# Villen-Lab/pyAscore

Measured on AMD Instinct MI355X. Metric: PSMs/sec (Ascore.score) at 1/2/4/8 MI355X + HBM-roofline %, higher is better.
Workload: dtype f32/f64 scalar + i32 counts

## Files before the change

pyascore_amd/csrc/common.h:

```cpp
#ifndef PYA_COMMON_H
#define PYA_COMMON_H

#include <stdint.h>

#define PYA_WAVE 64
#define PYA_NTOP 10
#define PYA_NTOP_MAX 16
#define PYA_NO_MATCH 15
#define PYA_TABLE_PAD 4
#define PYA_MAX_L 64
#define PYA_MAX_TYPES 8
#define PYA_MAX_NL 8
#define PYA_FAST_NL 4
#define PYA_MAX_UNIQ_WIDE 48
#define PYA_MAX_NL_CANDS 44
#define PYA_MAX_UNIQ 16
#define PYA_MAX_LIST 2048
#define PYA_MAX_LUT_N 4096
#define PYA_MAX_PUSHED 128

#define PYA_ST_OK 0
#define PYA_ST_NO_BINS 1
#define PYA_ST_TOO_MANY_BINS 2
#define PYA_ST_LUT_RANGE 3
#define PYA_ST_PUSHED_OVERFLOW 4
#define PYA_ST_ROUTE_CAPS 5
#define PYA_ST_INVALID 16
#define PYA_ST_OVER_LIMIT 17

struct PcCaps {
    uint32_t cap, pos_cap, kc, k_cap, n_cap;
};
// ... 117 lines not shown
```

pyascore_amd/csrc/fused_core.hip.h:

```cpp
#ifndef PYA_FUSED_CORE_H
#define PYA_FUSED_CORE_H
#include "score_core.hip.h"
#include "localize_core.hip.h"

#define FUSED_ROUND 3

struct FusedLds {
    uint16_t *grid;
    uint4 *cum_lut;
    PeakEntry *peaks;
    float2 *resd;
    uint8_t *rkl;
    uint32_t *rec;
    float *wsl;
    float *mass_l;
    uint32_t *flag_l;
    uint8_t *site_pos;
    float *selm;
    unsigned char *sort_raw;
    PushedEntry *pushed;
    unsigned long long *site_alt;
    uint32_t *site_max, *site_tie, *n_pushed;
    float *sc;
    uint32_t *c_tr, *c_cnt;
// ... 2 lines not shown
    float *srt_v;
    uint8_t *srt_h;
    int32_t *c_depth;
    uint32_t *c_site;
};

__host__ __device__ static inline size_t fused_align16(size_t v) { return (v + 15) & ~(size_t)15; }
__host__ __device__ static inline size_t fused_sort_bytes(uint32_t n) {
    if (n <= 64) return ((size_t)n * 10 + 15) & ~(size_t)15;
    return (((size_t)n * 6 + 15) & ~(size_t)15) + ((size_t)n / 64 + 2) * 16 + 2 * 128 * 2;
}
__host__ __device__ static inline uint32_t fused_site_cap(uint32_t push_cap) {
    const uint32_t v = (push_cap + 3u) & ~3u;
    return v > 64u ? 64u : (v < 4u ? 4u : v);
}
__host__ __device__ static inline size_t fused_post_bytes(uint32_t n_cap, uint32_t push_cap, uint32_t ent_cap, uint32_t ndir,
                                                          bool multi_z) {
    return fused_align16(fused_sort_bytes(n_cap)) + (size_t)push_cap * 16 + (size_t)fused_site_cap(push_cap) * 16 + 16 +
           (size_t)(1 + FUSED_ROUND) * 40 + (size_t)FUSED_ROUND * (16 * ndir + 4 + 4) + 16 + 64 +
           (multi_z ? fused_align16((size_t)FUSED_ROUND * ndir * 2 * ent_cap * 4) +
                          fused_align16((size_t)FUSED_ROUND * ndir * 2 * ent_cap)
                    : 0);
}
__host__ __device__ static inline size_t fused_walk_bytes(uint32_t cap) {
    return 16 * 16 + ((size_t)cap + PYA_TABLE_PAD) * 8;
}
__host__ __device__ static inline size_t fused_kept_bytes(uint32_t n_cap, uint32_t stride, uint32_t pos_cap, uint32_t ent_cap,
                                                          uint32_t ndir) {
    return fused_align16(((size_t)pos_cap + 1) * 8) + fused_align16((size_t)ent_cap * stride) + (size_t)n_cap * 16 + 256 +
           fused_align16((size_t)pos_cap + 1) + (size_t)(1 + FUSED_ROUND) * ndir * ent_cap * 4;
}
__host__ __device__ static inline size_t fused_lds_bytes(uint32_t cap, uint32_t n_cap, uint32_t stride, uint32_t pos_cap,
                                                         uint32_t ent_cap, uint32_t push_cap, uint32_t ndir, bool multi_z) {
    const size_t walk = fused_walk_bytes(cap), post = fused_post_bytes(n_cap, push_cap, ent_cap, ndir, multi_z);
    return PYA_GRID_CELLS * 2 + fused_align16(walk > post ? walk : post) +
           fused_kept_bytes(n_cap, stride, pos_cap, ent_cap, ndir) + 16;
}

DEV FusedLds fused_carve(unsigned char *raw, uint32_t cap, uint32_t n_cap, uint32_t stride, uint32_t pos_cap,
                         uint32_t ent_cap, uint32_t push_cap, uint32_t ndir, bool multi_z) {
    FusedLds f;
    f.grid = (uint16_t *)raw;
    size_t o = PYA_GRID_CELLS * 2;
    f.cum_lut = (uint4 *)(raw + o);
    f.peaks = (PeakEntry *)(raw + o + 16 * 16);
    f.sort_raw = raw + o;
    size_t q = o + fused_align16(fused_sort_bytes(n_cap));
    f.pushed = (PushedEntry *)(raw + q);
    q += (size_t)push_cap * sizeof(PushedEntry);
    const size_t sc = fused_site_cap(push_cap);
    f.site_alt = (unsigned long long *)(raw + q);
    q += sc * 8;
    f.site_max = (uint32_t *)(raw + q);
    q += sc * 4;
    f.site_tie = (uint32_t *)(raw + q);
    q += sc * 4;
    f.n_pushed = (uint32_t *)(raw + q);
    q += 16;
    f.sc = (float *)(raw + q);
    q += (size_t)(1 + FUSED_ROUND) * 40;
    f.c_tr = (uint32_t *)(raw + q);
    q += (size_t)FUSED_ROUND * ndir * 8;
    f.c_cnt = (uint32_t *)(raw + q);
    q += (size_t)FUSED_ROUND * ndir * 8;
    f.c_depth = (int32_t *)(raw + q);
    q += FUSED_ROUND * 4;
    f.c_site = (uint32_t *)(raw + q);
    q += FUSED_ROUND * 4;
    f.bad_tasks = (uint32_t *)(raw + q);
    q += 16;
    f.t_lo = (uint32_t *)(raw + q);
    f.t_off = f.t_lo + 8;
    q += 64;
    f.srt_v = (float *)(raw + q);
    q += fused_align16((size_t)FUSED_ROUND * ndir * 2 * ent_cap * 4);
    f.srt_h = (uint8_t *)(raw + q);
    const size_t walk = fused_walk_bytes(cap), post = fused_post_bytes(n_cap, push_cap, ent_cap, ndir, multi_z);
    o += fused_align16(walk > post ? walk : post);
    f.resd = (float2 *)(raw + o);
    o += fused_align16(((size_t)pos_cap + 1) * 8);
    f.rkl = (uint8_t *)(raw + o);
    o += fused_align16((size_t)ent_cap * stride);
    f.rec = (uint32_t *)(raw + o);
    o += (size_t)n_cap * 12;
    f.wsl = (float *)(raw + o);
    o += (size_t)n_cap * 4;
    f.mass_l = (float *)(raw + o);
    f.flag_l = (uint32_t *)(raw + o + 128);
    f.site_pos = (uint8_t *)(raw + o + 256);
    f.selm = (float *)(raw + o + 256 + fused_align16((size_t)pos_cap + 1));
    return f;
}


template <bool BZ>
DEV void walk_record_steps(const float2 *&rp, int rstride, StepBits &bits, float &running, const uint4 *lut, CumCounts &cum,
                           const PeakTable &tab, int zmax, double A, double B, uint8_t *&ro, int stride, int count) {
    for (int i = 0; i < count; i++, rp += rstride) {
        const float2 mm = *rp;
        running = (bits.next() ? mm.y : mm.x) + running;
// ... 86 lines not shown
DEV int partners_in_run(const float *run, int n, int p2, float me, int side, float err) {
    int j = 0;
    for (int step = p2 >> 1; step > 0; step >>= 1) {
        const int probe = j + step;
        const float o = probe - 1 < n ? run[probe - 1] : __builtin_huge_valf();
        const float dd = side ? (o - me) : (me - o);
        if (side ? (dd <= -err) : (dd >= err)) j = probe;
    }
    int cnt = 0;
    for (int q = j; q < j + 2 && q < n; q++) {
        const float dd = side ? (run[q] - me) : (me - run[q]);
        cnt += (__builtin_fabsf(dd) < err) ? 1 : 0;
    }
    return cnt;
}

#define FUSED_LOCAL_CHUNKS 8
struct LocalTable {
    const float *mz;
    const uint8_t *rank;
    int R, status;
};

template <bool BOTH, bool ZM, bool WIDE = false>
DEV bool fused_body(const BatchDev &b, uint32_t psm, unsigned char *lds_raw, uint32_t cap, uint32_t n_cap, uint32_t stride,
                    uint32_t pos_cap, uint32_t ent_cap, uint32_t push_cap, const LocalTable *local = nullptr) {
    const int lane = lane_id();
    const DevConfig *cfg = b.cfg;
    const int ndir = BOTH ? 2 : 1;
    const FusedLds f = fused_carve(lds_raw, cap, n_cap, stride, pos_cap, ent_cap, push_cap, (uint32_t)ndir, ZM);
    STAMP_BEGIN();
    STAMP_T(b, 38, false);
    float lmz[FUSED_LOCAL_CHUNKS];
    uint32_t lrk[FUSED_LOCAL_CHUNKS];
    if (local) {
#pragma unroll
        for (int q = 0; q < FUSED_LOCAL_CHUNKS; q++) {
            const int i = q * 64 + lane_id();
            lmz[q] = i < local->R ? local->mz[i] : __builtin_huge_valf();
            lrk[q] = i < local->R ? (uint32_t)local->rank[i] : (uint32_t)PYA_NO_MATCH;
        }
        wave_lds_sync();
    }
    if (lane < 32) {
        f.mass_l[lane] = cfg->res_mass[lane];
        f.flag_l[lane] = cfg->res_modifiable[lane];
    }
    const uint64_t *dw = b.desc + (size_t)psm * PYA_DESC_WORDS;
    const int64_t p0 = (int64_t)dw[0], pep0 = (int64_t)dw[1], s0 = (int64_t)dw[2], a0 = (int64_t)dw[3];
    const uint64_t w4 = dw[4], w5 = dw[5];
    const int L = (int)(w4 & 0xffffu), n_aux = (int)((w4 >> 16) & 0xffffu), k = (int)((w4 >> 32) & 0xffffu);
    const int zmax = ZM ? (int)(w4 >> 56) : 1;
    const int N = (int)(uint32_t)w5;
    const uint64_t *order = b.order_tab + (uint32_t)(w5 >> 32);
    const int status = local ? local->status : b.status[psm];
    const int R = local ? local->R : (int)b.ret_n[psm];

    const uint32_t max_k = b.max_k;
    float *out_asc = b.ascores + (size_t)psm * max_k;
    uint64_t *out_alt = b.alt_mask + (size_t)psm * max_k;
    for (uint32_t a = lane; a < max_k; a += 64) {
        out_asc[a] = 0.f;
        out_alt[a] = 0ull;
    }
    if (status != PYA_ST_OK) {
        if (lane == 0) {
            b.best_score[psm] = -1.f;
            b.best_sig[psm] = 0ull;
            b.n_sig_out[psm] = -1;
        }
        return false;
    }
    STAMP_T(b, 39, false);
    const bool two_pass = BOTH && WIDE && N > 32;
    const int s = (BOTH && !two_pass) ? (lane & 31) : lane;
    const int dir = BOTH ? (two_pass ? 0 : (lane >> 5)) : (cfg->n_fwd > 0 ? 0 : 1);
    const bool active = s < N;
    const uint32_t letter = lane < L ? (uint32_t)b.pep[pep0 + lane] : (uint32_t)'A';
    const uint64_t bits = active ? order[s] : 0ull;
// ... 541 lines not shown
```

pyascore_amd/csrc/host_internal.h:

```cpp
#ifndef PYA_HOST_INTERNAL_H
#define PYA_HOST_INTERNAL_H
#include <hip/hip_runtime_api.h>

#include <algorithm>
#include <atomic>
#include <cmath>
#include <cstdarg>
#include <cstddef>
#include <cstdio>
#include <cstdlib>
#include <chrono>
#include <cstring>
#include <condition_variable>
#include <functional>
#include <map>
#include <memory>
#include <mutex>
#include <string>
#include <thread>
#include <unordered_map>
#include <vector>

#include "../../include/pyascore_hip.h"
#include "common.h"
// ... 31 lines not shown
                   uint32_t use_fused, uint32_t f_n_cap, uint32_t f_stride, uint32_t f_ent_cap, uint32_t f_push_cap,
                   uint32_t multi_z, int32_t *host_status, uint32_t *host_flag, hipStream_t stream);
int pya_launch_ambiguity(const BatchDev *b, uint32_t psm, uint32_t peak_cap, uint32_t list_cap,
                         uint64_t ref_bits, uint64_t oth_bits, const float *d_scores, float ref_ws,
                         float oth_ws, float *d_out, hipStream_t stream);
int pya_launch_debug_sort(const float *d_keys, uint32_t n, uint32_t *d_perm, hipStream_t stream);
int pya_launch_pack_records(const float *best_score, const int32_t *n_sig, const uint64_t *best_sig, const float *ascores,
                            const uint64_t *alt_mask, uint32_t k, uint32_t res_k, uint64_t n_psm, int32_t *out, hipStream_t stream);
int pya_launch_debug_wave_ops(const int32_t *d_in, int32_t *d_out, hipStream_t stream);
size_t pya_score_big_lds_bytes(uint32_t cap, uint32_t pos_cap, uint32_t kc);
int pya_launch_score_big(const BatchDev *b, const uint32_t *d_ids, uint32_t n_ids, uint32_t cap, uint32_t pos_cap, uint32_t kc,
                         uint32_t inline_on, hipStream_t stream);
size_t pya_localize_recount_lds_bytes(uint32_t cap, uint32_t push_cap, uint32_t pos_cap, uint32_t pool_cap, uint32_t sb);
size_t pya_localize_hash_lds_bytes(uint32_t push_cap, uint32_t n_cap, uint32_t pos_cap, uint32_t sb, uint32_t vc, uint32_t hs,
                                   uint32_t pp, uint32_t max_k, uint32_t n_nl);
int pya_launch_localize_hash(const BatchDev *b, const uint32_t *d_ids, uint32_t n_ids, uint32_t push_cap, uint32_t n_cap,
                             uint32_t pos_cap, uint32_t pool_cap, uint32_t sb, uint32_t gtp, uint32_t vc, uint32_t hs, uint32_t pp,
                             uint32_t n_nl, hipStream_t stream);
int pya_launch_localize_recount(const BatchDev *b, const uint32_t *d_ids, uint32_t n_ids, uint32_t cap, uint32_t push_cap,
                                uint32_t pos_cap, uint32_t pool_cap, uint32_t sb, uint32_t gtp, uint32_t *d_redo_count, uint32_t *d_redo_ids, hipStream_t stream);
int pya_launch_score_big_list(const BatchDev *b, const uint32_t *d_count, const uint32_t *d_ids, uint32_t n_max, uint32_t cap,
                              uint32_t pos_cap, uint32_t kc, hipStream_t stream);
uint32_t pya_big_inline_max(void);
size_t pya_fused_lds_bytes(uint32_t cap, uint32_t n_cap, uint32_t stride, uint32_t pos_cap, uint32_t ent_cap, uint32_t push_cap,
                           uint32_t both, uint32_t multi_z);
int pya_launch_fused(const BatchDev *b, const uint32_t *d_ids, uint32_t n_ids, uint32_t cap, uint32_t n_cap,
                     uint32_t stride, uint32_t pos_cap, uint32_t ent_cap, uint32_t push_cap, uint32_t both,
                     uint32_t multi_z, uint32_t *d_redo_count, uint32_t *d_redo_ids, hipStream_t stream);
size_t pya_score_cnt_lds_bytes(uint32_t cap, uint32_t pos_cap, uint32_t kc, uint32_t k_cap, uint32_t n_cap);
int pya_launch_score_cnt(const BatchDev *b, const uint32_t *d_ids, uint32_t n_ids, uint32_t cap, uint32_t pos_cap, uint32_t kc, uint32_t k_cap,
                         uint32_t n_cap, hipStream_t stream);
size_t pya_score_cntg_lds_bytes(uint32_t cap, uint32_t pos_cap, uint32_t k_cap, uint32_t n_cap, uint32_t nl_cap);
int pya_launch_score_cntg(const BatchDev *b, const uint32_t *d_ids, uint32_t n_ids, uint32_t cap, uint32_t pos_cap, uint32_t k_cap, uint32_t n_cap,
                          uint32_t nl_cap, hipStream_t stream);
size_t pya_bin_global_scratch_bytes(uint32_t cap);
int pya_launch_bin_global(const BatchDev *b, const uint32_t *d_ids, uint32_t n_ids, unsigned char *d_scratch, uint64_t stride,
                          uint32_t cap, uint32_t types, hipStream_t stream);
size_t pya_general_lds_bytes(uint32_t l_cap, uint32_t list_cap);
size_t pya_general_scratch_bytes(uint32_t n_cap, uint32_t push_cap);
int pya_launch_general(const BatchDev *b, const uint32_t *d_ids, uint32_t n_ids, unsigned char *d_scratch, const uint64_t *d_scratch_off,
                       uint32_t l_cap, uint32_t list_cap, hipStream_t stream);
int pya_launch_general_ambiguity(const BatchDev *b, uint32_t psm, uint32_t l_cap, uint32_t list_cap, uint64_t ref_bits,
                                 uint64_t oth_bits, const float *d_scores, uint32_t n_scores, float ref_ws, float oth_ws,
                                 float *d_out, hipStream_t stream);
size_t pya_evidence_lds_bytes(uint32_t l_cap, uint32_t list_cap);
int pya_launch_evidence(const BatchDev *b, const uint32_t *d_ids, uint32_t n_ids, void *d_out, uint32_t l_cap, uint32_t list_cap,
                        hipStream_t stream);
size_t pya_ions_lds_bytes(uint32_t l_cap, uint32_t list_cap);
uint32_t pya_ions_scan_tiles(uint32_t n);
int pya_launch_ions(const BatchDev *b, const uint32_t *d_ids, uint32_t n_ids, const void *d_evid, int64_t *d_off, void *d_out, uint64_t cap,
// ... 128 lines not shown
        case 'C': return 103.00919f;  case 'L': return 113.08406f;  case 'I': return 113.08406f;
        case 'N': return 114.04293f;  case 'D': return 115.02694f;  case 'Q': return 128.05858f;
        case 'K': return 128.09496f;  case 'E': return 129.04259f;  case 'M': return 131.04049f;
        case 'H': return 137.05891f;  case 'F': return 147.06841f;  case 'U': return 150.95364f;
        case 'R': return 156.10111f;  case 'Y': return 163.06333f;  case 'W': return 186.07931f;
        case 'O': return 237.14773f;
    }
    return 0.f;
}


struct Knobs {
    bool no_plain = false, no_fused = false, no_big = false, no_tiny = false, no_prefix = false, no_chunks = false;
    bool no_upload_thread = false, one_peak_class = false, peak_classes = false, one_lds_class = false;
    bool host_timing = false, stamps = false, sort_room = false, no_big_inline = false;
    bool no_loc_hash = false, no_nodes = false, no_cnt = false, no_prob_cnt = false;
    bool no_fork = false;
    bool slow_null_stream = false;
    uint32_t debug = 0;
    int64_t plain_min = 512, big_min_n = 1024, tiny_max = 64;
    int64_t bin_select_min = 640;
    int64_t bin_select_scap = 768;
    uint32_t sort_room_max = 1024;
    int sb = -1, gtp = -1, hash_pp = -1;
    int node_cap = -1;
    double chunk_mb = 0.;
    int64_t workspace_mb = 0;
};

void read_knobs(Knobs &k);
bool set_knob(Knobs &k, const char *key, const char *value);

struct pya_handle {
    Knobs kn;
    int device = 0;
    hipStream_t side_stream = nullptr;
    float bin_size = 100.f, mod_mass = 0.f, mz_error = 0.5f;
    uint32_t n_top = PYA_NTOP;
    uint32_t rec_words() const { return (n_top + 1u) / 2u + 1u; }
    std::string mod_group, fragment_types;
    std::map<char, float> nl;
    DevConfig cfg;
    bool cfg_dirty = true;
    DevBuf<DevConfig> d_cfg;

    std::vector<float> lut;
// ... 287 lines not shown
    DevBuf<uint32_t> d_sret_n;
    DevBuf<int32_t> d_sstatus;
    uint64_t spec(uint64_t i) const { return spec_of.empty() ? i : spec_of[i]; }
    int64_t n_peaks(uint64_t i) const {
        const uint64_t s = spec(i);
        return peak_off[s + 1] - peak_off[s];
    }
    DevBuf<uint16_t> d_grid;
    DevBuf<uint32_t> d_redo3;
    DevBuf<uint32_t> d_redo;
    Bucket buckets[kNumBuckets];
    struct IdList {
        uint32_t off, n, cap, ncls;
    };
    static bool any_ids(const std::vector<IdList> &lists) {
        bool any = false;
        for (const IdList &l : lists) any = any || l.n != 0;
        return any;
    }
    std::vector<uint32_t> bin_ids, score_ids, fused_ids, big_ids;
    std::vector<IdList> bin_lists, score_lists, big_lists;
    struct FusedLaunch {
        uint32_t off, n, cap, multi_z, n_cap, stride, pos_cap, ent_cap, push_cap;
    };
    std::vector<FusedLaunch> fused_launches;
    uint32_t n_fused_total = 0;
    std::vector<uint8_t> gen;
    std::vector<uint32_t> gen_ids;
    DevBuf<uint32_t> d_gen_ids;
    DevBuf<unsigned char> d_gen_scratch;
    uint32_t gen_l_cap = 1, gen_list_cap = 1;
    std::vector<uint64_t> gen_off;
    DevBuf<uint64_t> d_gen_off;
    std::vector<uint32_t> bigbin_ids;
    DevBuf<uint32_t> d_bigbin_ids;
    DevBuf<unsigned char> d_bigbin_scratch;
    uint32_t bigbin_cap = 32;
    size_t bigbin_stride = 0;
    std::vector<uint8_t> big;
    DevBuf<uint32_t> d_big_ids;
    uint32_t big_pos_cap = 1, big_k_max = 1;
    uint32_t big_kc() const {
        uint32_t v = 8u;
        while (v < big_k_max + 1u) v <<= 1;
        return v;
    }
// ... 270 lines not shown
```

pyascore_amd/csrc/host_plan.cpp:

```cpp
#include "host_internal.h"

int check_psm_shape(const pya_handle *h, uint64_t i, int64_t P, int64_t L, int32_t k, int32_t z, const uint8_t *pep,
                    const uint32_t *aux_pos, int64_t n_aux, uint32_t *ns, char *msg) {
    const unsigned long long iu = i;
    auto say = [msg](int code, const char *fmt, auto... args) {
        std::snprintf(msg, kPsmMsg, fmt, args...);
        return code;
    };
    if (P <= 0) return say(PYA_ERR_PSM, "PSM %llu: empty spectrum", iu);
    if (P > PYA_MAX_PEAKS) return say(PYA_ERR_LIMIT, "PSM %llu: %lld peaks exceed the limit of %d", iu, (long long)P, PYA_MAX_PEAKS);
    if (L < 1 || L > PYA_MAX_PEPTIDE_LEN)
        return say(L < 1 ? PYA_ERR_PSM : PYA_ERR_LIMIT, "PSM %llu: peptide length %lld outside 1..%d", iu, (long long)L, PYA_MAX_PEPTIDE_LEN);
    if (k < 0) return say(PYA_ERR_PSM, "PSM %llu: negative n_of_mod", iu);
    if (z < 1 || z > PYA_MAX_CHARGE)
        return say(z < 1 ? PYA_ERR_PSM : PYA_ERR_LIMIT, "PSM %llu: max_fragment_charge %d outside 1..%d", iu, z, PYA_MAX_CHARGE);
    if (n_aux < 0) return say(PYA_ERR_ARG, "PSM %llu: aux_off is not monotone", iu);
    uint32_t cnt = 0;
    int64_t bad_j = -1, bad_a = -1;
    for (int64_t j = 0; j < L; j++) {
        if (!h->is_residue[pep[j]] && bad_j < 0) bad_j = j;
        if (h->letter_modifiable((char)pep[j], (size_t)j, (size_t)L)) cnt++;
    }
    for (int64_t a = 0; a < n_aux; a++)
        if (aux_pos[a] > (uint32_t)L && bad_a < 0) bad_a = a;
// ... 386 lines not shown
        if (key != last_key) {
            auto it = std::lower_bound(keys.begin(), keys.end(), std::make_pair(key, 0u));
            if (it == keys.end() || it->first != key) {
                it = keys.insert(it, std::make_pair(key, (uint32_t)cnt.size()));
                cnt.push_back(0);
            }
            last_key = key;
            last_cls = it->second;
        }
        cls[t] = last_cls;
        cnt[last_cls]++;
    }
    std::vector<size_t> at(cnt.size());
    size_t acc = 0;
    for (const auto &kc : keys) {
        at[kc.second] = acc;
        acc += cnt[kc.second];
    }
    std::vector<FusedItem> sorted(items.size());
    for (size_t t = 0; t < items.size(); t++) sorted[at[cls[t]]++] = items[t];
    items.swap(sorted);
}

void fused_launches(PlanBuild &B) {
    pya_plan *p = B.p;
    const uint32_t ndir = B.both_dirs ? 2u : 1u;
    std::vector<FusedItem> items;
    for (uint64_t i = 0; i < B.n; i++) {
        if (!p->fused[i] || p->pre_status[i]) continue;
        FusedItem it;
        it.id = (uint32_t)i;
        const uint32_t z = (uint32_t)p->max_charge[i], Lm1 = (uint32_t)(p->pep_off[i + 1] - p->pep_off[i] - 1);
        const uint32_t kk = (uint32_t)p->n_of_mod[i], ns = p->n_sites[i];
        it.group = (uint32_t)B.pcls[i] * 2 + (z > 1 ? 1u : 0u);
        it.n_cap = (p->n_sig[i] + 3u) & ~3u;
        it.pos = std::max(Lm1, 1u);
        it.ent = std::max(Lm1 * z, 1u);
        it.push = std::min<uint32_t>(PYA_MAX_PUSHED, (kk * (ns - kk) + 7u) & ~7u);
        if (it.push < 8) it.push = 8;
        it.need = pya_fused_lds_bytes(B.caps[B.pcls[i]], it.n_cap, ndir * it.n_cap + 4, it.pos, it.ent, it.push, p->fused_both, z > 1 ? 1u : 0u);
        items.push_back(it);
    }
    p->n_fused_total = (uint32_t)items.size();
    sort_fused_items(items);
    p->fused_ids.resize(items.size());
    size_t g0 = 0;
    while (g0 < items.size()) {
        size_t g1 = g0;
        while (g1 < items.size() && items[g1].group == items[g0].group) g1++;
        std::vector<size_t> cuts{g0};
        if (g1 - g0 >= 8192 && !B.h->kn.one_lds_class) {
            const size_t need_max = items[g1 - 1].need;
            for (double q : {0.5, 0.85}) {
                const size_t at = g0 + (size_t)(q * (double)(g1 - g0));
                size_t cut = at;
                while (cut < g1 && items[cut].need == items[at].need) cut++;
                if (cut < g1 && cut > cuts.back() && items[at].need * 5 <= need_max * 4) cuts.push_back(cut);
            }
        }
        cuts.push_back(g1);
        for (size_t c = 0; c + 1 < cuts.size(); c++) {
            pya_plan::FusedLaunch fl = {(uint32_t)cuts[c], (uint32_t)(cuts[c + 1] - cuts[c]), B.caps[items[g0].group / 2],
                                        items[g0].group & 1u, 4, 4, 1, 1, 8};
            for (size_t t = cuts[c]; t < cuts[c + 1]; t++) {
                fl.n_cap = std::max(fl.n_cap, items[t].n_cap);
                fl.pos_cap = std::max(fl.pos_cap, items[t].pos);
                fl.ent_cap = std::max(fl.ent_cap, items[t].ent);
                fl.push_cap = std::max(fl.push_cap, items[t].push);
                p->fused_ids[t] = items[t].id;
            }
            fl.stride = ndir * fl.n_cap + 4;
            p->fused_launches.push_back(fl);
        }
        g0 = g1;
    }
}

void pack_descriptors(PlanBuild &B) {
    pya_plan *p = B.p;
    p->desc.resize((size_t)B.n * PYA_DESC_WORDS);
    for (uint64_t i = 0; i < B.n; i++) {
        uint64_t *w = &p->desc[(size_t)i * PYA_DESC_WORDS];
        const uint64_t L = (uint64_t)std::max<int64_t>(0, std::min<int64_t>(p->pep_off[i + 1] - p->pep_off[i], 0xffff));
        const uint64_t na = (uint64_t)std::max<int64_t>(0, std::min<int64_t>(p->aux_off[i + 1] - p->aux_off[i], 0xffff));
        w[0] = (uint64_t)p->ret_off[i];
        w[1] = (uint64_t)p->pep_off[i];
// ... 347 lines not shown
```

pyascore_amd/csrc/host_run.cpp:

```cpp
#include "host_internal.h"

namespace {

struct ScoreRoute {
    enum Kind { kCountNodes, kCountNodesGeneral, kSignatures } kind;
    uint32_t prefix, compact, kc, node_cap, node_cols, res_cap, nl_cap;
};

ScoreRoute pick_score_route(const pya_handle *h, const Bucket &bk, uint32_t ncls, uint32_t peak_cap) {
    const DevConfig &c = h->cfg;
    ScoreRoute r = {ScoreRoute::kSignatures, score_prefix(h, bk.n_cap), score_compact(c, bk.z_max), 8u, 0u, 0u, 0u, nl_cap(c)};
    const bool general = general_settings(c);
    const bool cnt_ok = h->mz_error <= 0.49f && bk.k_max + 1u <= 31u && bk.ns_max <= 32u && !h->kn.no_cnt && !(h->kn.debug & 0x8000u);
    if (ncls >= 1 && !general && c.n_fwd == 1 && c.n_types == 2 && bk.z_max == 1 && cnt_ok) {
        while (r.kc < bk.k_max + 1u) r.kc <<= 1;
        if (pya_score_cnt_lds_bytes(peak_cap, bk.pos_cap, r.kc, bk.k_max, bk.ns_max) <= 64u * 1024u) {
            r.kind = ScoreRoute::kCountNodes;
            return r;
        }
    }
    if (general && cnt_ok && pya_score_cntg_lds_bytes(peak_cap, bk.pos_cap, bk.k_max, bk.ns_max, r.nl_cap) <= 64u * 1024u) {
        r.kind = ScoreRoute::kCountNodesGeneral;
        return r;
    }
// ... 60 lines not shown
    }
    e = pya_launch_bin_exact(&d, (uint32_t)p->n_psm, p->peak_cap, types, st);
    if (e) return h->hip_fail((hipError_t)e, "bin_spectra (exact) launch");
    e = pya_launch_bin_global(&d, p->d_bigbin_ids.p, (uint32_t)p->bigbin_ids.size(), p->d_bigbin_scratch.p, p->bigbin_stride, p->bigbin_cap, types, st);
    if (e) return h->hip_fail((hipError_t)e, "bin_spectra (global) launch");
    return PYA_OK;
}

int run_binning_shared(pya_plan *p, const BatchDev &d, uint32_t types, hipStream_t st) {
    BatchDev sd = d;
    sd.ret_off = p->d_sret_off.p;
    sd.ret_n = p->d_sret_n.p;
    sd.status = p->d_sstatus.p;
    const int rc = run_binning(p, sd, types, st);
    if (rc) return rc;
    const int e = pya_launch_fan_out(p->d_spec_of.p, p->d_sret_n.p, p->d_sstatus.p, d.ret_n, d.status, (uint32_t)p->n_psm, st);
    if (e) return p->h->hip_fail((hipError_t)e, "fan-out launch");
    return PYA_OK;
}

int run_fused_family(pya_plan *p, const BatchDev &d, hipStream_t fs) {
    pya_handle *h = p->h;
    const Bucket &fb = p->fusedb;
    for (const pya_plan::FusedLaunch &l : p->fused_launches) {
        int fe = pya_launch_fused(&d, p->d_fused_ids.p + l.off, l.n, l.cap, l.n_cap, l.stride, l.pos_cap, l.ent_cap, l.push_cap,
                                  p->fused_both, l.multi_z, d.redo4_count, d.redo4_ids, fs);
        if (fe) return h->hip_fail((hipError_t)fe, "score_localize launch");
    }
    int fe = pya_launch_localize_redo(&d, d.redo4_count, d.redo4_ids, p->n_fused_total, fb.push_cap(), fb.n_cap,
                                      fb.pos_cap, fb.pool_cap(), fb.sb(), fb.gtp(), fs);
    if (fe) return h->hip_fail((hipError_t)fe, "localize (hand-over) launch");
    return PYA_OK;
}

int run_scoring(pya_plan *p, const BatchDev &d, hipStream_t st) {
    pya_handle *h = p->h;
    int e = 0;
    for (const pya_plan::IdList &l : p->score_lists) {
        const Bucket &bk = p->buckets[l.ncls];
        const uint32_t *ids = p->d_score_ids.p + l.off;
        const ScoreRoute r = pick_score_route(h, bk, l.ncls, l.cap);
        switch (r.kind) {
            case ScoreRoute::kCountNodes:
                e = pya_launch_score_cnt(&d, ids, l.n, l.cap, bk.pos_cap, r.kc, bk.k_max, bk.ns_max, st);
                if (e) return h->hip_fail((hipError_t)e, "score_cnt launch");
                break;
            case ScoreRoute::kCountNodesGeneral:
                e = pya_launch_score_cntg(&d, ids, l.n, l.cap, bk.pos_cap, bk.k_max, bk.ns_max, r.nl_cap, st);
                if (e) return h->hip_fail((hipError_t)e, "score_cntg launch");
                break;
            case ScoreRoute::kSignatures:
// ... 852 lines not shown
```

pyascore_amd/csrc/host_tables.cpp:

```cpp
#include "host_internal.h"

static void read_env(Knobs &k) {
    auto flag = [](const char *n) { return std::getenv(n) != nullptr; };
    k.host_timing = flag("PYA_HOST_TIMING");
    k.stamps = flag("PYA_STAMPS");
    k.chunk_mb = 0.;
    if (const char *e = std::getenv("PYA_CHUNK_MB")) k.chunk_mb = std::max(1.0, std::atof(e));
    const char *w = std::getenv("PYA_WORKSPACE_MB");
    k.workspace_mb = w ? (int64_t)std::atoll(w) : 0;
}

void read_knobs(Knobs &k) {
    k = Knobs();
    read_env(k);
}

bool set_knob(Knobs &k, const char *key, const char *value) {
    const Knobs dflt;
    const std::string name(key ? key : "");
    const bool on = value != nullptr;
    auto num = [&](int64_t d) { return on ? (int64_t)std::strtoll(value, nullptr, 0) : d; };
    struct { const char *n; bool Knobs::*m; } flags[] = {
        {"PYA_NO_PLAIN", &Knobs::no_plain}, {"PYA_NO_FUSED", &Knobs::no_fused}, {"PYA_NO_BIG", &Knobs::no_big},
        {"PYA_NO_TINY", &Knobs::no_tiny}, {"PYA_NO_PREFIX", &Knobs::no_prefix}, {"PYA_NO_CHUNKS", &Knobs::no_chunks},
        {"PYA_NO_UPLOAD_THREAD", &Knobs::no_upload_thread}, {"PYA_ONE_PEAK_CLASS", &Knobs::one_peak_class},
        {"PYA_PEAK_CLASSES", &Knobs::peak_classes}, {"PYA_ONE_LDS_CLASS", &Knobs::one_lds_class},
        {"PYA_SORT_ROOM", &Knobs::sort_room}, {"PYA_NO_BIG_INLINE", &Knobs::no_big_inline},
        {"PYA_NO_LOC_HASH", &Knobs::no_loc_hash}, {"PYA_NO_CNT", &Knobs::no_cnt}, {"PYA_NO_PROB_CNT", &Knobs::no_prob_cnt}, {"PYA_NO_NODES", &Knobs::no_nodes},
        {"PYA_HOST_TIMING", &Knobs::host_timing}, {"PYA_STAMPS", &Knobs::stamps},
        {"PYA_SLOW_NULL_STREAM", &Knobs::slow_null_stream}, {"PYA_NO_FORK", &Knobs::no_fork},
    };
    bool known = false;
    for (auto &f : flags)
        if (name == f.n) {
            k.*(f.m) = on;
            known = true;
        }
    if (name == "PYA_DEBUG") k.debug = (uint32_t)num(0), known = true;
    else if (name == "PYA_PLAIN_MIN") k.plain_min = num(dflt.plain_min), known = true;
    else if (name == "PYA_BIG_MIN_N") k.big_min_n = num(dflt.big_min_n), known = true;
    else if (name == "PYA_BIN_SELECT_MIN") k.bin_select_min = num(dflt.bin_select_min), known = true;
    else if (name == "PYA_BIN_SELECT_SCAP") k.bin_select_scap = num(dflt.bin_select_scap), known = true;
    else if (name == "PYA_TINY_MAX") k.tiny_max = num(dflt.tiny_max), known = true;
    else if (name == "PYA_SORT_ROOM_MAX") k.sort_room_max = (uint32_t)num(dflt.sort_room_max), known = true;
    else if (name == "PYA_SB") k.sb = (int)num(-1), known = true;
    else if (name == "PYA_GTP") k.gtp = (int)num(-1), known = true;
    else if (name == "PYA_HASH_PP") k.hash_pp = (int)num(-1), known = true;
    else if (name == "PYA_NODE_CAP") k.node_cap = (int)num(-1), known = true;
    else if (name == "PYA_CHUNK_MB") k.chunk_mb = on ? std::max(1.0, std::atof(value)) : 0., known = true;
    else if (name == "PYA_WORKSPACE_MB") k.workspace_mb = num(0), known = true;
    return known;
}


int build_dev_config(pya_handle *h) {
    DevConfig &c = h->cfg;
    std::memset(&c, 0, sizeof c);
    c.bin_size = h->bin_size;
    c.mod_mass = h->mod_mass;
    c.mz_error = h->mz_error;
    int nt = 0;
    for (char t : h->fragment_types)
        if (is_forward(t)) c.types[nt++] = (uint8_t)t;
    c.n_fwd = nt;
    for (char t : h->fragment_types)
        if (is_backward(t)) c.types[nt++] = (uint8_t)t;
    c.n_types = nt;
// ... 207 lines not shown
```

pyascore_amd/csrc/score_localize.hip:

```cpp
#include "fused_core.hip.h"

#ifndef FUSED_WAVES
#define FUSED_WAVES 6
#endif

template <bool BOTH, bool ZM, bool WIDE = false>
__global__ __launch_bounds__(64, FUSED_WAVES) void pya_score_localize_kernel(
    BatchDev b, const uint32_t *psm_ids, uint32_t n_ids, uint32_t cap, uint32_t n_cap, uint32_t stride, uint32_t pos_cap,
    uint32_t ent_cap, uint32_t push_cap, uint32_t *redo_count, uint32_t *redo_ids) {
    extern __shared__ __attribute__((aligned(16))) unsigned char lds_raw[];
    if (blockIdx.x >= n_ids) return;
    const uint32_t psm = psm_ids[xcd_slot(blockIdx.x, n_ids)];
    const bool declined = fused_body<BOTH, ZM, WIDE>(b, psm, lds_raw, cap, n_cap, stride, pos_cap, ent_cap, push_cap);
    if (declined && lane_id() == 0) redo_ids[atomicAdd(redo_count, 1u)] = psm;
}

extern "C" size_t pya_fused_lds_bytes(uint32_t cap, uint32_t n_cap, uint32_t stride, uint32_t pos_cap, uint32_t ent_cap,
                                      uint32_t push_cap, uint32_t both, uint32_t multi_z) {
    return fused_lds_bytes(cap, n_cap, stride, pos_cap, ent_cap, push_cap, both ? 2u : 1u, multi_z != 0);
}

extern "C" int pya_launch_fused(const BatchDev *b, const uint32_t *d_ids, uint32_t n_ids, uint32_t cap, uint32_t n_cap,
                                uint32_t stride, uint32_t pos_cap, uint32_t ent_cap, uint32_t push_cap, uint32_t both,
                                uint32_t multi_z, uint32_t *d_redo_count, uint32_t *d_redo_ids, hipStream_t stream) {
    if (n_ids == 0) return 0;
    const size_t lds = fused_lds_bytes(cap, n_cap, stride, pos_cap, ent_cap, push_cap, both ? 2u : 1u, multi_z != 0);
#define PYA_FUSED_LAUNCH(B, Z, W)                                                                                          \
    do {                                                                                                                   \
        hipError_t e = PYA_ENSURE_MAX_LDS((pya_score_localize_kernel<B, Z, W>));                                           \
        if (e != hipSuccess) return (int)e;                                                                                \
        hipLaunchKernelGGL((pya_score_localize_kernel<B, Z, W>), dim3(n_ids), dim3(64), lds, stream, *b, d_ids, n_ids, cap, \
                           n_cap, stride, pos_cap, ent_cap, push_cap, d_redo_count, d_redo_ids);                           \
    } while (0)
    const bool wide = both && n_cap > 32u;
    if (both && multi_z && wide) PYA_FUSED_LAUNCH(true, true, true);
    else if (both && wide) PYA_FUSED_LAUNCH(true, false, true);
    else if (both && multi_z) PYA_FUSED_LAUNCH(true, true, false);
    else if (both) PYA_FUSED_LAUNCH(true, false, false);
    else if (multi_z) PYA_FUSED_LAUNCH(false, true, false);
    else PYA_FUSED_LAUNCH(false, false, false);
#undef PYA_FUSED_LAUNCH
    return (int)hipGetLastError();
}
```

pyascore_amd/csrc/tiny_batch.hip:

```cpp
#include "bin_core.hip.h"
#include "score_core.hip.h"
#include "localize_body.hip.h"
#include "fused_core.hip.h"

__global__ __launch_bounds__(64) void pya_tiny_batch_kernel(BatchDev b, uint32_t n_psm, uint32_t cap, uint32_t prefix,
                                                            uint32_t with_nl, uint32_t compact, uint32_t push_cap,
                                                            uint32_t pos_cap, uint32_t pool_cap, uint32_t sb,
                                                            uint32_t gtp) {
    extern __shared__ __attribute__((aligned(16))) unsigned char lds_raw[];
    const uint32_t psm = blockIdx.x;
    if (psm >= n_psm) return;
    {
        const float *r_mz;
        const uint8_t *r_rank;
        int status;
        int R = bin_core<false>(b, psm, lds_raw, cap, &r_mz, &r_rank, &status);
        if (R == PYA_BIN_REDO) {
            wave_lds_sync();
            R = bin_core<true>(b, psm, lds_raw, cap, &r_mz, &r_rank, &status);
        }
        bin_store(b, psm, R, status, r_mz, r_rank);
    }
    __threadfence();
    wave_lds_sync();
// ... 55 lines not shown
    }
    if (lane < 6) ((uint64_t *)b.desc)[lane] = m.desc[lane];
    if (lane < PYA_MAX_L / 8) ((uint64_t *)b.pep)[lane] = m.pep[lane];
    if (lane < PYA_ONE_MAX_AUX) {
        ((uint32_t *)b.aux_pos)[lane] = m.aux_pos[lane];
        ((float *)b.aux_mass)[lane] = m.aux_mass[lane];
    }
    __threadfence();
    wave_lds_sync();
    const uint64_t tk1 = __builtin_amdgcn_s_memrealtime();
    const float *r_mz;
    const uint8_t *r_rank;
    int bin_status;
    int R = bin_fast<false, true>(b, 0, lds_raw, cap, &r_mz, &r_rank, &bin_status, &pre);
    if (R == PYA_BIN_REDO) {
        wave_lds_sync();
        R = bin_core<true>(b, 0, lds_raw, cap, &r_mz, &r_rank, &bin_status);
    }
    bin_store(b, 0, R, bin_status, r_mz, r_rank);
    const uint64_t tk2 = __builtin_amdgcn_s_memrealtime();
    bool general = use_fused == 0;
    if (!general && R <= FUSED_LOCAL_CHUNKS * 64 - PYA_TABLE_PAD) {
        LocalTable lt = {r_mz, r_rank, R < 0 ? 0 : R, R < 0 ? bin_status : PYA_ST_OK};
        const bool declined = use_fused == 1 ? fused_body<true, ZM>(b, 0, lds_raw, cap, f_n_cap, f_stride, pos_cap, f_ent_cap, f_push_cap, &lt)
                                             : fused_body<false, ZM>(b, 0, lds_raw, cap, f_n_cap, f_stride, pos_cap, f_ent_cap, f_push_cap, &lt);
        general = declined;
    } else {
        __threadfence();
        wave_lds_sync();
        if (!general) {
            const bool declined = use_fused == 1 ? fused_body<true, ZM>(b, 0, lds_raw, cap, f_n_cap, f_stride, pos_cap, f_ent_cap, f_push_cap)
                                                 : fused_body<false, ZM>(b, 0, lds_raw, cap, f_n_cap, f_stride, pos_cap, f_ent_cap, f_push_cap);
            general = declined;
        } else {
            if (prefix) score_body<true>(b, 0, lds_raw, cap, with_nl, compact);
            else score_body<false>(b, 0, lds_raw, cap, with_nl, 0u);
        }
    }
    const uint64_t tk3 = __builtin_amdgcn_s_memrealtime();
    if (general) {
        __threadfence();
        wave_lds_sync();
        localize_body<false>(b, 0, lds_raw, push_cap, pos_cap, pool_cap, sb, gtp);
    }
    __threadfence_system();
    wave_lds_sync();
    if (lane == 0) {
        host_status[0] = b.status[0];
        host_status[1] = (int32_t)m.seq;
        host_status[2] = (int32_t)(tk1 - tk0);
        host_status[3] = (int32_t)(tk2 - tk1);
        host_status[4] = (int32_t)(tk3 - tk2);
        host_status[5] = (int32_t)(__builtin_amdgcn_s_memrealtime() - tk3);
        host_status[6] = (int32_t)(__builtin_amdgcn_s_memtime() - cy0);
        __threadfence_system();
// ... 33 lines not shown
```

Baseline: 205.2 million.

## Split fused score-localize into small-LDS first pass and full-cap second pass

The fused score/localize kernel now sizes its walk LDS region from a reduced return-table cap (default 224, rounded to 32) when the bin cap is large. PSMs whose binned table does not fit skip the first launch and are handled by a second launch at full cap over the same id list. The smaller LDS footprint is meant to raise occupancy for the common case. The cost is a second launch over every id and an extra early-exit check in each block.

```diff
diff --git a/pyascore_amd/csrc/common.h b/pyascore_amd/csrc/common.h
--- a/pyascore_amd/csrc/common.h
+++ b/pyascore_amd/csrc/common.h
@@ -8,6 +8,8 @@
 #define PYA_NTOP_MAX 16
 #define PYA_NO_MATCH 15
 #define PYA_TABLE_PAD 4
+#define PYA_FUSED_RET_BUDGET 224
+#define PYA_FUSED_RET_MIN_CAP 512
 #define PYA_MAX_L 64
 #define PYA_MAX_TYPES 8
 #define PYA_MAX_NL 8
diff --git a/pyascore_amd/csrc/fused_core.hip.h b/pyascore_amd/csrc/fused_core.hip.h
--- a/pyascore_amd/csrc/fused_core.hip.h
+++ b/pyascore_amd/csrc/fused_core.hip.h
@@ -48,22 +48,22 @@
                           fused_align16((size_t)FUSED_ROUND * ndir * 2 * ent_cap)
                     : 0);
 }
-__host__ __device__ static inline size_t fused_walk_bytes(uint32_t cap) {
-    return 16 * 16 + ((size_t)cap + PYA_TABLE_PAD) * 8;
+__host__ __device__ static inline size_t fused_walk_bytes(uint32_t ret_cap) {
+    return 16 * 16 + ((size_t)ret_cap + PYA_TABLE_PAD) * 8;
 }
 __host__ __device__ static inline size_t fused_kept_bytes(uint32_t n_cap, uint32_t stride, uint32_t pos_cap, uint32_t ent_cap,
                                                           uint32_t ndir) {
     return fused_align16(((size_t)pos_cap + 1) * 8) + fused_align16((size_t)ent_cap * stride) + (size_t)n_cap * 16 + 256 +
            fused_align16((size_t)pos_cap + 1) + (size_t)(1 + FUSED_ROUND) * ndir * ent_cap * 4;
 }
-__host__ __device__ static inline size_t fused_lds_bytes(uint32_t cap, uint32_t n_cap, uint32_t stride, uint32_t pos_cap,
+__host__ __device__ static inline size_t fused_lds_bytes(uint32_t ret_cap, uint32_t n_cap, uint32_t stride, uint32_t pos_cap,
                                                          uint32_t ent_cap, uint32_t push_cap, uint32_t ndir, bool multi_z) {
-    const size_t walk = fused_walk_bytes(cap), post = fused_post_bytes(n_cap, push_cap, ent_cap, ndir, multi_z);
+    const size_t walk = fused_walk_bytes(ret_cap), post = fused_post_bytes(n_cap, push_cap, ent_cap, ndir, multi_z);
     return PYA_GRID_CELLS * 2 + fused_align16(walk > post ? walk : post) +
            fused_kept_bytes(n_cap, stride, pos_cap, ent_cap, ndir) + 16;
 }
 
-DEV FusedLds fused_carve(unsigned char *raw, uint32_t cap, uint32_t n_cap, uint32_t stride, uint32_t pos_cap,
+DEV FusedLds fused_carve(unsigned char *raw, uint32_t ret_cap, uint32_t n_cap, uint32_t stride, uint32_t pos_cap,
                          uint32_t ent_cap, uint32_t push_cap, uint32_t ndir, bool multi_z) {
     FusedLds f;
     f.grid = (uint16_t *)raw;
@@ -101,7 +101,7 @@
     f.srt_v = (float *)(raw + q);
     q += fused_align16((size_t)FUSED_ROUND * ndir * 2 * ent_cap * 4);
     f.srt_h = (uint8_t *)(raw + q);
-    const size_t walk = fused_walk_bytes(cap), post = fused_post_bytes(n_cap, push_cap, ent_cap, ndir, multi_z);
+    const size_t walk = fused_walk_bytes(ret_cap), post = fused_post_bytes(n_cap, push_cap, ent_cap, ndir, multi_z);
     o += fused_align16(walk > post ? walk : post);
     f.resd = (float2 *)(raw + o);
     o += fused_align16(((size_t)pos_cap + 1) * 8);
@@ -234,13 +234,14 @@
     int R, status;
 };
 
-template <bool BOTH, bool ZM, bool WIDE = false>
-DEV bool fused_body(const BatchDev &b, uint32_t psm, unsigned char *lds_raw, uint32_t cap, uint32_t n_cap, uint32_t stride,
-                    uint32_t pos_cap, uint32_t ent_cap, uint32_t push_cap, const LocalTable *local = nullptr) {
+template <bool BOTH, bool ZM, bool WIDE = false, bool TWO = false>
+DEV bool fused_body(const BatchDev &b, uint32_t psm, unsigned char *lds_raw, uint32_t cap, uint32_t ret_cap, uint32_t ret_lo,
+                    uint32_t n_cap, uint32_t stride, uint32_t pos_cap, uint32_t ent_cap, uint32_t push_cap,
+                    const LocalTable *local = nullptr) {
     const int lane = lane_id();
     const DevConfig *cfg = b.cfg;
     const int ndir = BOTH ? 2 : 1;
-    const FusedLds f = fused_carve(lds_raw, cap, n_cap, stride, pos_cap, ent_cap, push_cap, (uint32_t)ndir, ZM);
+    const FusedLds f = fused_carve(lds_raw, ret_cap, n_cap, stride, pos_cap, ent_cap, push_cap, (uint32_t)ndir, ZM);
     STAMP_BEGIN();
     STAMP_T(b, 38, false);
     float lmz[FUSED_LOCAL_CHUNKS];
@@ -267,6 +268,10 @@
     const uint64_t *order = b.order_tab + (uint32_t)(w5 >> 32);
     const int status = local ? local->status : b.status[psm];
     const int R = local ? local->R : (int)b.ret_n[psm];
+    if (TWO) {
+        const uint32_t need = (uint32_t)R + PYA_TABLE_PAD;
+        if (ret_lo ? (status != PYA_ST_OK || need <= ret_lo) : (status == PYA_ST_OK && ret_cap < cap && need > ret_cap)) return false;
+    }
 
     const uint32_t max_k = b.max_k;
     float *out_asc = b.ascores + (size_t)psm * max_k;
diff --git a/pyascore_amd/csrc/host_internal.h b/pyascore_amd/csrc/host_internal.h
--- a/pyascore_amd/csrc/host_internal.h
+++ b/pyascore_amd/csrc/host_internal.h
@@ -77,10 +77,12 @@
 int pya_launch_score_big_list(const BatchDev *b, const uint32_t *d_count, const uint32_t *d_ids, uint32_t n_max, uint32_t cap,
                               uint32_t pos_cap, uint32_t kc, hipStream_t stream);
 uint32_t pya_big_inline_max(void);
-size_t pya_fused_lds_bytes(uint32_t cap, uint32_t n_cap, uint32_t stride, uint32_t pos_cap, uint32_t ent_cap, uint32_t push_cap,
+size_t pya_fused_lds_bytes(uint32_t ret_cap, uint32_t n_cap, uint32_t stride, uint32_t pos_cap, uint32_t ent_cap, uint32_t push_cap,
                            uint32_t both, uint32_t multi_z);
-int pya_launch_fused(const BatchDev *b, const uint32_t *d_ids, uint32_t n_ids, uint32_t cap, uint32_t n_cap,
-                     uint32_t stride, uint32_t pos_cap, uint32_t ent_cap, uint32_t push_cap, uint32_t both,
+void pya_fused_lds_parts(uint32_t ret_cap, uint32_t n_cap, uint32_t stride, uint32_t pos_cap, uint32_t ent_cap, uint32_t push_cap,
+                         uint32_t both, uint32_t multi_z, size_t parts[4]);
+int pya_launch_fused(const BatchDev *b, const uint32_t *d_ids, uint32_t n_ids, uint32_t cap, uint32_t ret_cap, uint32_t ret_lo,
+                     uint32_t n_cap, uint32_t stride, uint32_t pos_cap, uint32_t ent_cap, uint32_t push_cap, uint32_t both,
                      uint32_t multi_z, uint32_t *d_redo_count, uint32_t *d_redo_ids, hipStream_t stream);
 size_t pya_score_cnt_lds_bytes(uint32_t cap, uint32_t pos_cap, uint32_t kc, uint32_t k_cap, uint32_t n_cap);
 int pya_launch_score_cnt(const BatchDev *b, const uint32_t *d_ids, uint32_t n_ids, uint32_t cap, uint32_t pos_cap, uint32_t kc, uint32_t k_cap,
@@ -255,6 +257,7 @@
     int64_t bin_select_min = 640;
     int64_t bin_select_scap = 768;
     uint32_t sort_room_max = 1024;
+    int64_t fused_ret_cap = -1;
     int sb = -1, gtp = -1, hash_pp = -1;
     int node_cap = -1;
     double chunk_mb = 0.;
@@ -588,6 +591,7 @@
     std::vector<IdList> bin_lists, score_lists, big_lists;
     struct FusedLaunch {
         uint32_t off, n, cap, multi_z, n_cap, stride, pos_cap, ent_cap, push_cap;
+        uint32_t ret_cap;
     };
     std::vector<FusedLaunch> fused_launches;
     uint32_t n_fused_total = 0;
diff --git a/pyascore_amd/csrc/host_plan.cpp b/pyascore_amd/csrc/host_plan.cpp
--- a/pyascore_amd/csrc/host_plan.cpp
+++ b/pyascore_amd/csrc/host_plan.cpp
@@ -432,6 +432,12 @@
     items.swap(sorted);
 }
 
+uint32_t fused_ret_cap(const pya_handle *h, uint32_t cap) {
+    if (h->kn.fused_ret_cap < 0 && cap < PYA_FUSED_RET_MIN_CAP) return cap;
+    const int64_t v = std::min<int64_t>(h->kn.fused_ret_cap < 0 ? PYA_FUSED_RET_BUDGET : h->kn.fused_ret_cap, (int64_t)cap);
+    return std::min(cap, ((uint32_t)v + 31u) & ~31u);
+}
+
 void fused_launches(PlanBuild &B) {
     pya_plan *p = B.p;
     const uint32_t ndir = B.both_dirs ? 2u : 1u;
@@ -448,7 +454,7 @@
         it.ent = std::max(Lm1 * z, 1u);
         it.push = std::min<uint32_t>(PYA_MAX_PUSHED, (kk * (ns - kk) + 7u) & ~7u);
         if (it.push < 8) it.push = 8;
-        it.need = pya_fused_lds_bytes(B.caps[B.pcls[i]], it.n_cap, ndir * it.n_cap + 4, it.pos, it.ent, it.push, p->fused_both, z > 1 ? 1u : 0u);
+        it.need = pya_fused_lds_bytes(fused_ret_cap(B.h, B.caps[B.pcls[i]]), it.n_cap, ndir * it.n_cap + 4, it.pos, it.ent, it.push, p->fused_both, z > 1 ? 1u : 0u);
         items.push_back(it);
     }
     p->n_fused_total = (uint32_t)items.size();
@@ -471,7 +477,8 @@
         cuts.push_back(g1);
         for (size_t c = 0; c + 1 < cuts.size(); c++) {
             pya_plan::FusedLaunch fl = {(uint32_t)cuts[c], (uint32_t)(cuts[c + 1] - cuts[c]), B.caps[items[g0].group / 2],
-                                        items[g0].group & 1u, 4, 4, 1, 1, 8};
+                                        items[g0].group & 1u, 4, 4, 1, 1, 8, 0};
+            fl.ret_cap = fused_ret_cap(B.h, fl.cap);
             for (size_t t = cuts[c]; t < cuts[c + 1]; t++) {
                 fl.n_cap = std::max(fl.n_cap, items[t].n_cap);
                 fl.pos_cap = std::max(fl.pos_cap, items[t].pos);
diff --git a/pyascore_amd/csrc/host_run.cpp b/pyascore_amd/csrc/host_run.cpp
--- a/pyascore_amd/csrc/host_run.cpp
+++ b/pyascore_amd/csrc/host_run.cpp
@@ -106,11 +106,14 @@
 int run_fused_family(pya_plan *p, const BatchDev &d, hipStream_t fs) {
     pya_handle *h = p->h;
     const Bucket &fb = p->fusedb;
-    for (const pya_plan::FusedLaunch &l : p->fused_launches) {
-        int fe = pya_launch_fused(&d, p->d_fused_ids.p + l.off, l.n, l.cap, l.n_cap, l.stride, l.pos_cap, l.ent_cap, l.push_cap,
-                                  p->fused_both, l.multi_z, d.redo4_count, d.redo4_ids, fs);
-        if (fe) return h->hip_fail((hipError_t)fe, "score_localize launch");
-    }
+    for (int pass = 0; pass < 2; pass++)
+        for (const pya_plan::FusedLaunch &l : p->fused_launches) {
+            if (pass && l.ret_cap >= l.cap) continue;
+            int fe = pya_launch_fused(&d, p->d_fused_ids.p + l.off, l.n, l.cap, pass ? l.cap : l.ret_cap, pass ? l.ret_cap : 0u,
+                                      l.n_cap, l.stride, l.pos_cap, l.ent_cap, l.push_cap, p->fused_both, l.multi_z, d.redo4_count,
+                                      d.redo4_ids, fs);
+            if (fe) return h->hip_fail((hipError_t)fe, pass ? "score_localize (second pass) launch" : "score_localize launch");
+        }
     int fe = pya_launch_localize_redo(&d, d.redo4_count, d.redo4_ids, p->n_fused_total, fb.push_cap(), fb.n_cap,
                                       fb.pos_cap, fb.pool_cap(), fb.sb(), fb.gtp(), fs);
     if (fe) return h->hip_fail((hipError_t)fe, "localize (hand-over) launch");
diff --git a/pyascore_amd/csrc/host_tables.cpp b/pyascore_amd/csrc/host_tables.cpp
--- a/pyascore_amd/csrc/host_tables.cpp
+++ b/pyascore_amd/csrc/host_tables.cpp
@@ -43,6 +43,7 @@
     else if (name == "PYA_BIN_SELECT_SCAP") k.bin_select_scap = num(dflt.bin_select_scap), known = true;
     else if (name == "PYA_TINY_MAX") k.tiny_max = num(dflt.tiny_max), known = true;
     else if (name == "PYA_SORT_ROOM_MAX") k.sort_room_max = (uint32_t)num(dflt.sort_room_max), known = true;
+    else if (name == "PYA_FUSED_RET_CAP") k.fused_ret_cap = on ? std::max<int64_t>(0, num(0)) : -1, known = true;
     else if (name == "PYA_SB") k.sb = (int)num(-1), known = true;
     else if (name == "PYA_GTP") k.gtp = (int)num(-1), known = true;
     else if (name == "PYA_HASH_PP") k.hash_pp = (int)num(-1), known = true;
diff --git a/pyascore_amd/csrc/score_localize.hip b/pyascore_amd/csrc/score_localize.hip
--- a/pyascore_amd/csrc/score_localize.hip
+++ b/pyascore_amd/csrc/score_localize.hip
@@ -4,33 +4,50 @@
 #define FUSED_WAVES 6
 #endif
 
-template <bool BOTH, bool ZM, bool WIDE = false>
+template <bool BOTH, bool ZM, bool WIDE, bool TWO>
 __global__ __launch_bounds__(64, FUSED_WAVES) void pya_score_localize_kernel(
-    BatchDev b, const uint32_t *psm_ids, uint32_t n_ids, uint32_t cap, uint32_t n_cap, uint32_t stride, uint32_t pos_cap,
-    uint32_t ent_cap, uint32_t push_cap, uint32_t *redo_count, uint32_t *redo_ids) {
+    BatchDev b, const uint32_t *psm_ids, uint32_t n_ids, uint32_t cap, uint32_t ret_cap, uint32_t ret_lo, uint32_t n_cap,
+    uint32_t stride, uint32_t pos_cap, uint32_t ent_cap, uint32_t push_cap, uint32_t *redo_count, uint32_t *redo_ids) {
     extern __shared__ __attribute__((aligned(16))) unsigned char lds_raw[];
     if (blockIdx.x >= n_ids) return;
     const uint32_t psm = psm_ids[xcd_slot(blockIdx.x, n_ids)];
-    const bool declined = fused_body<BOTH, ZM, WIDE>(b, psm, lds_raw, cap, n_cap, stride, pos_cap, ent_cap, push_cap);
+    const bool declined = fused_body<BOTH, ZM, WIDE, TWO>(b, psm, lds_raw, cap, ret_cap, ret_lo, n_cap, stride, pos_cap, ent_cap, push_cap);
     if (declined && lane_id() == 0) redo_ids[atomicAdd(redo_count, 1u)] = psm;
 }
 
-extern "C" size_t pya_fused_lds_bytes(uint32_t cap, uint32_t n_cap, uint32_t stride, uint32_t pos_cap, uint32_t ent_cap,
+extern "C" size_t pya_fused_lds_bytes(uint32_t ret_cap, uint32_t n_cap, uint32_t stride, uint32_t pos_cap, uint32_t ent_cap,
                                       uint32_t push_cap, uint32_t both, uint32_t multi_z) {
-    return fused_lds_bytes(cap, n_cap, stride, pos_cap, ent_cap, push_cap, both ? 2u : 1u, multi_z != 0);
+    return fused_lds_bytes(ret_cap, n_cap, stride, pos_cap, ent_cap, push_cap, both ? 2u : 1u, multi_z != 0);
 }
 
-extern "C" int pya_launch_fused(const BatchDev *b, const uint32_t *d_ids, uint32_t n_ids, uint32_t cap, uint32_t n_cap,
-                                uint32_t stride, uint32_t pos_cap, uint32_t ent_cap, uint32_t push_cap, uint32_t both,
-                                uint32_t multi_z, uint32_t *d_redo_count, uint32_t *d_redo_ids, hipStream_t stream) {
+extern "C" void pya_fused_lds_parts(uint32_t ret_cap, uint32_t n_cap, uint32_t stride, uint32_t pos_cap, uint32_t ent_cap,
+                                    uint32_t push_cap, uint32_t both, uint32_t multi_z, size_t parts[4]) {
+    const uint32_t ndir = both ? 2u : 1u;
+    parts[0] = PYA_GRID_CELLS * 2;
+    parts[1] = fused_walk_bytes(ret_cap);
+    parts[2] = fused_post_bytes(n_cap, push_cap, ent_cap, ndir, multi_z != 0);
+    parts[3] = fused_kept_bytes(n_cap, stride, pos_cap, ent_cap, ndir);
+}
+
+extern "C" int pya_launch_fused(const BatchDev *b, const uint32_t *d_ids, uint32_t n_ids, uint32_t cap, uint32_t ret_cap,
+                                uint32_t ret_lo, uint32_t n_cap, uint32_t stride, uint32_t pos_cap, uint32_t ent_cap,
+                                uint32_t push_cap, uint32_t both, uint32_t multi_z, uint32_t *d_redo_count, uint32_t *d_redo_ids,
+                                hipStream_t stream) {
     if (n_ids == 0) return 0;
-    const size_t lds = fused_lds_bytes(cap, n_cap, stride, pos_cap, ent_cap, push_cap, both ? 2u : 1u, multi_z != 0);
+    if (ret_cap > cap || (ret_lo && ret_cap != cap)) return (int)hipErrorInvalidValue;
+    const size_t lds = fused_lds_bytes(ret_cap, n_cap, stride, pos_cap, ent_cap, push_cap, both ? 2u : 1u, multi_z != 0);
+    const bool two = ret_cap < cap || ret_lo != 0;
+#define PYA_FUSED_LAUNCH_T(B, Z, W, T)                                                                                     \
+    do {                                                                                                                   \
+        hipError_t e = PYA_ENSURE_MAX_LDS((pya_score_localize_kernel<B, Z, W, T>));                                        \
+        if (e != hipSuccess) return (int)e;                                                                                \
+        hipLaunchKernelGGL((pya_score_localize_kernel<B, Z, W, T>), dim3(n_ids), dim3(64), lds, stream, *b, d_ids, n_ids,  \
+                           cap, ret_cap, ret_lo, n_cap, stride, pos_cap, ent_cap, push_cap, d_redo_count, d_redo_ids);     \
+    } while (0)
 #define PYA_FUSED_LAUNCH(B, Z, W)                                                                                          \
     do {                                                                                                                   \
-        hipError_t e = PYA_ENSURE_MAX_LDS((pya_score_localize_kernel<B, Z, W>));                                           \
-        if (e != hipSuccess) return (int)e;                                                                                \
-        hipLaunchKernelGGL((pya_score_localize_kernel<B, Z, W>), dim3(n_ids), dim3(64), lds, stream, *b, d_ids, n_ids, cap, \
-                           n_cap, stride, pos_cap, ent_cap, push_cap, d_redo_count, d_redo_ids);                           \
+        if (two) PYA_FUSED_LAUNCH_T(B, Z, W, true);                                                                        \
+        else PYA_FUSED_LAUNCH_T(B, Z, W, false);                                                                           \
     } while (0)
     const bool wide = both && n_cap > 32u;
     if (both && multi_z && wide) PYA_FUSED_LAUNCH(true, true, true);
@@ -40,5 +57,6 @@
     else if (multi_z) PYA_FUSED_LAUNCH(false, true, false);
     else PYA_FUSED_LAUNCH(false, false, false);
 #undef PYA_FUSED_LAUNCH
+#undef PYA_FUSED_LAUNCH_T
     return (int)hipGetLastError();
 }
diff --git a/pyascore_amd/csrc/tiny_batch.hip b/pyascore_amd/csrc/tiny_batch.hip
--- a/pyascore_amd/csrc/tiny_batch.hip
+++ b/pyascore_amd/csrc/tiny_batch.hip
@@ -101,15 +101,15 @@
     bool general = use_fused == 0;
     if (!general && R <= FUSED_LOCAL_CHUNKS * 64 - PYA_TABLE_PAD) {
         LocalTable lt = {r_mz, r_rank, R < 0 ? 0 : R, R < 0 ? bin_status : PYA_ST_OK};
-        const bool declined = use_fused == 1 ? fused_body<true, ZM>(b, 0, lds_raw, cap, f_n_cap, f_stride, pos_cap, f_ent_cap, f_push_cap, &lt)
-                                             : fused_body<false, ZM>(b, 0, lds_raw, cap, f_n_cap, f_stride, pos_cap, f_ent_cap, f_push_cap, &lt);
+        const bool declined = use_fused == 1 ? fused_body<true, ZM>(b, 0, lds_raw, cap, cap, 0u, f_n_cap, f_stride, pos_cap, f_ent_cap, f_push_cap, &lt)
+                                             : fused_body<false, ZM>(b, 0, lds_raw, cap, cap, 0u, f_n_cap, f_stride, pos_cap, f_ent_cap, f_push_cap, &lt);
         general = declined;
     } else {
         __threadfence();
         wave_lds_sync();
         if (!general) {
-            const bool declined = use_fused == 1 ? fused_body<true, ZM>(b, 0, lds_raw, cap, f_n_cap, f_stride, pos_cap, f_ent_cap, f_push_cap)
-                                                 : fused_body<false, ZM>(b, 0, lds_raw, cap, f_n_cap, f_stride, pos_cap, f_ent_cap, f_push_cap);
+            const bool declined = use_fused == 1 ? fused_body<true, ZM>(b, 0, lds_raw, cap, cap, 0u, f_n_cap, f_stride, pos_cap, f_ent_cap, f_push_cap)
+                                                 : fused_body<false, ZM>(b, 0, lds_raw, cap, cap, 0u, f_n_cap, f_stride, pos_cap, f_ent_cap, f_push_cap);
             general = declined;
         } else {
             if (prefix) score_body<true>(b, 0, lds_raw, cap, with_nl, compact);
```

Result: no change. 203.9 million (-0.6%).
